# lucasjinreal/yolov7_d2

Hardware: NVIDIA H100
Metric: images/sec (640x640) YOLOX-s fwd+bwd (higher is better)
Workload: dtype bf16

## Files before the change

yolov7_d2_b200/csrc/conv_api.cu:

```cuda
#include "conv_gemm.cuh"
#include "host_common.cuh"
#include "wgrad_gemm.cuh"

#include <algorithm>
#include <cstring>

namespace yb {

template <int BN, int BK>
static int launch_conv_inst(const CUtensorMap& tmA, const CUtensorMap& tmB, const ConvGemmParams& p, dim3 grid, cudaStream_t st) {
  using Cfg = ConvGemmCfg<BN, BK>;
  const bool ext = p.epi_mode >= EPI_BF16_AFFINE;
  const int phases = p.num_phases == 4 ? 4 : 1;
  const int m_tiles = grid.x * phases, n_tiles = grid.y;
  const int occ = conv_min_ctas(BN, BK);
  const bool xpose = p.epi_mode == EPI_F32_BIAS && p.out_sc == 1;
  const int fixed = ConvEpiCfg<BN>::kStageBytes + (xpose ? kXposeBytes : 0);
  const int budget = (occ == 1 ? 212 : 104) * 1024 - 1024 - fixed;
  int slots_kb = budget / Cfg::kStageBytes;
  const int num_kb = phases == 4 ? p.cin_blocks : p.num_taps * p.cin_blocks;
  int kbs = 1;
  if (BK <= 32)
    for (int t = 1; t <= num_kb; ++t)
      if (num_kb % t == 0 && t * BK <= 144 && 2 * t <= slots_kb) kbs = t;
  int pst = slots_kb / kbs;
  if (pst > kMaxStagesP) pst = kMaxStagesP;
  if (pst < 2) pst = 2;
  const int smem = pst * kbs * Cfg::kStageBytes + 1024 + fixed;
  static PerDevice<int> smem_limit(0);
  YB_CHECK_CUDA(raise_smem_limit(smem_limit, smem, conv_gemm_persistent_kernel<BN, BK, false>, conv_gemm_persistent_kernel<BN, BK, true>));
  int groups = (occ * sm_count()) / n_tiles;
  if (groups < 1) groups = 1;
  if (groups > m_tiles) groups = m_tiles;
  if (phases == 4 && groups > 1 && groups % 2 == 0) --groups;
  ConvGemmParams pp = p;
  pp.xpose = xpose ? 1 : 0;
  if (ext)
    launch_k(conv_gemm_persistent_kernel<BN, BK, true>, groups * n_tiles, kConvThreadsP, smem, st, tmA, tmB, pp, pst, kbs, n_tiles, m_tiles);
  else
    launch_k(conv_gemm_persistent_kernel<BN, BK, false>, groups * n_tiles, kConvThreadsP, smem, st, tmA, tmB, pp, pst, kbs, n_tiles, m_tiles);
  YB_CHECK_CUDA(cudaGetLastError());
  return 0;
}

static int launch_conv(int bn, int bk, const CUtensorMap& tmA, const CUtensorMap& tmB, const ConvGemmParams& p, dim3 grid, cudaStream_t st) {
#define YB_CASE(BN, BK) \
  if (bn == BN && bk == BK) return launch_conv_inst<BN, BK>(tmA, tmB, p, grid, st);
  YB_CASE(16, 16) YB_CASE(16, 32) YB_CASE(16, 64)
  YB_CASE(32, 16) YB_CASE(32, 32) YB_CASE(32, 64)
  YB_CASE(64, 16) YB_CASE(64, 32) YB_CASE(64, 64)
  YB_CASE(128, 16) YB_CASE(128, 32) YB_CASE(128, 64)
#undef YB_CASE
  return fail(YB200_ERR_UNSUPPORTED, "no conv_gemm instantiation for BLOCK_N=%d BLOCK_K=%d", bn, bk);
}

static int pick_block_k(int c) { return c % 64 == 0 ? 64 : (c % 32 == 0 ? 32 : (c % 16 == 0 ? 16 : 0)); }
static int pick_block_n(int c) { return c > 64 ? 128 : (c > 32 ? 64 : (c > 16 ? 32 : 16)); }

static int check_arg(const yb200_act* a, const char* who, const char* arg) {
  char name[96];
  snprintf(name, sizeof(name), "%s %s", who, arg);
  return check_act(a, name);
}

static int fill_fwd_taps(ConvTap* taps, const yb200_act& x, int ksize, int stride, int k_per_tap) {
  int nt = 0;
  if (ksize == 1) {
    taps[nt++] = ConvTap{x.c_off, 0, 0, 0, 0};
  } else if (ksize == 2) {
    for (int kh = 0; kh < 2; ++kh)
      for (int kw = 0; kw < 2; ++kw) taps[nt++] = ConvTap{kw * x.c_pitch + x.c_off, 0, kh, 0, (kh * 2 + kw) * k_per_tap};
  } else {
    for (int kh = 0; kh < 3; ++kh)
      for (int kw = 0; kw < 3; ++kw) {
        ConvTap t{};
        if (stride == 1) {
          t.c0 = x.c_off; t.dw = kw - 1; t.p = 0; t.dh = kh - 1;
        } else {
          t.p = (kh == 1) ? 0 : 1; t.dh = (kh == 0) ? -1 : 0;
          const int pw = (kw == 1) ? 0 : 1;
          t.dw = (kw == 0) ? -1 : 0;
          t.c0 = pw * x.c_pitch + x.c_off;
        }
        t.kb = (kh * 3 + kw) * k_per_tap;
        taps[nt++] = t;
      }
  }
  return nt;
}

static ConvGemmParams out_view(const yb200_act& o) {
  ConvGemmParams p;
  memset(&p, 0, sizeof(p));
  p.out = static_cast<__nv_bfloat16*>(o.ptr) + o.c_off;
  p.out_sw = o.c_pitch;
  p.out_sh = 1LL * o.c_pitch * o.w;
  p.out_sn = 1LL * o.c_pitch * o.w * o.h;
  p.out_sc = 1;
  p.out_mh = 1; p.out_mw = 1;
  return p;
}
static ConvGemmParams out_rows_f32(float* out, int w, int a_total, int a_off, int c_total, int c_off) {
  ConvGemmParams p;
  memset(&p, 0, sizeof(p));
  p.out = out + 1LL * a_off * c_total + c_off;
  p.out_sn = 1LL * a_total * c_total;
  p.out_sh = 1LL * w * c_total;
  p.out_sw = c_total;
  p.out_sc = 1;
  p.out_mh = 1; p.out_mw = 1;
  return p;
}
static ConvGemmParams out_nchw_f32(float* out, int cout, int h, int w) {
  ConvGemmParams p;
  memset(&p, 0, sizeof(p));
  const long long hw = 1LL * h * w;
  p.out = out;
  p.out_sn = 1LL * cout * hw;
  p.out_sh = w;
  p.out_sw = 1;
  p.out_sc = static_cast<int>(hw);
  p.out_mh = 1; p.out_mw = 1;
  return p;
}
static ConvGemmParams out_nhwc_f32(float* out, int pitch, int h, int w) {
  ConvGemmParams p;
  memset(&p, 0, sizeof(p));
  p.out = out;
  p.out_sw = pitch;
  p.out_sh = 1LL * pitch * w;
  p.out_sn = 1LL * pitch * w * h;
  p.out_sc = 1;
  p.out_mh = 1; p.out_mw = 1;
  return p;
}

static void set_addend(ConvGemmParams& p, const yb200_act* a) {
  p.addend = static_cast<const __nv_bfloat16*>(a->ptr) + a->c_off;
  p.add_sw = a->c_pitch;
  p.add_sh = 1LL * a->c_pitch * a->w;
  p.add_sn = 1LL * a->c_pitch * a->w * a->h;
}

static void set_tiles(ConvGemmParams& p, int n, int h, int w) {
  choose_tile(n, h, w, 128, &p.log_tw, &p.log_th);
  const int tw = 1 << p.log_tw, th = 1 << p.log_th, tn = 128 >> (p.log_tw + p.log_th);
  p.tiles_w = ceil_div(w, tw); p.tiles_h = ceil_div(h, th); p.tiles_n = ceil_div(n, tn);
  p.n_valid = n; p.h_valid = h; p.w_valid = w;
}

}

using namespace yb;

__global__ void pack_conv_weight_kernel(const float* __restrict__ w, const float* __restrict__ cout_scale, int cout, int cin, int taps, int cout_pad,
                                        int cin_pad, __nv_bfloat16* __restrict__ wf, __nv_bfloat16* __restrict__ wd) {
  pdl_sync();
  const long long total = 1LL * cout_pad * taps * cin_pad;
  for (long long i = blockIdx.x * (long long)blockDim.x + threadIdx.x; i < total; i += (long long)gridDim.x * blockDim.x) {
    const int ci = static_cast<int>(i % cin_pad);
    const int t = static_cast<int>((i / cin_pad) % taps);
    const int co = static_cast<int>(i / (1LL * cin_pad * taps));
    float v = (co < cout && ci < cin) ? w[(1LL * co * cin + ci) * taps + t] : 0.f;
    if (cout_scale != nullptr && co < cout) v *= cout_scale[co];
    const __nv_bfloat16 b = __float2bfloat16_rn(v);
    if (wf) wf[i] = b;
    if (wd) wd[(1LL * ci * taps + t) * cout_pad + co] = b;
  }
}

static int pack_weight_impl(const float* w_oihw, const float* cout_scale, int cout, int cin, int ksize, int cout_pad, int cin_pad, void* w_fwd,
                            void* w_dgrad, void* stream) {
  YB_REQUIRE(w_oihw && (w_fwd || w_dgrad), YB200_ERR_INVALID, "pack_conv_weight: null pointer");
  YB_REQUIRE(cout > 0 && cin > 0 && (ksize >= 1 && ksize <= 3) && cout_pad >= cout && cin_pad >= cin, YB200_ERR_INVALID,
             "pack_conv_weight: bad sizes cout=%d cin=%d k=%d pads=%d,%d", cout, cin, ksize, cout_pad, cin_pad);
  const long long total = 1LL * cout_pad * ksize * ksize * cin_pad;
  const int blocks = static_cast<int>(std::min<long long>((total + 255) / 256, 4096));
  launch_k(pack_conv_weight_kernel, blocks, 256, 0, as_stream(stream), w_oihw, cout_scale, cout, cin, ksize * ksize, cout_pad, cin_pad,
                                                                 static_cast<__nv_bfloat16*>(w_fwd),
                                                                 static_cast<__nv_bfloat16*>(w_dgrad));
  YB_CHECK_CUDA(cudaGetLastError());
  return 0;
}

constexpr int kPackMaxLayers = 256;
__global__ void __launch_bounds__(256)
pack_conv_weights_batched_kernel(const yb200_pack_desc* __restrict__ table, const long long* __restrict__ prefix, int n) {
  pdl_sync();
  __shared__ int s_rows[kPackMaxLayers + 1];
  if (threadIdx.x == 0) {
    int acc = 0;
    for (int l = 0; l < n; ++l) {
      s_rows[l] = acc;
      const yb200_pack_desc d = table[l];
      const int taps = d.ksize * d.ksize;
      acc += (d.w_fwd ? d.cout_pad * taps : 0) + (d.w_dgrad ? d.cin_pad * taps : 0);
    }
    s_rows[n] = acc;
  }
  __syncthreads();
  const int total_rows = s_rows[n];
  const int lane = threadIdx.x & 31;
  const int warps = (gridDim.x * blockDim.x) >> 5;
  for (int r = (blockIdx.x * blockDim.x + threadIdx.x) >> 5; r < total_rows; r += warps) {
    int lo = 0, hi = n - 1;
    while (lo < hi) {
      const int mid = (lo + hi + 1) >> 1;
      if (s_rows[mid] <= r) lo = mid; else hi = mid - 1;
    }
    const yb200_pack_desc d = table[lo];
    const int taps = d.ksize * d.ksize;
    int q = r - s_rows[lo];
    const int fwd_rows = d.w_fwd ? d.cout_pad * taps : 0;
    if (q < fwd_rows) {
      const int co = q / taps, t = q - co * taps;
      __nv_bfloat16* dst = static_cast<__nv_bfloat16*>(d.w_fwd) + static_cast<size_t>(q) * d.cin_pad;
      const float* src = d.w_oihw + static_cast<size_t>(co) * d.cin * taps + t;
      for (int ci = lane; ci < d.cin_pad; ci += 32)
        dst[ci] = __float2bfloat16_rn((co < d.cout && ci < d.cin) ? src[static_cast<size_t>(ci) * taps] : 0.f);
    } else {
      q -= fwd_rows;
      const int ci = q / taps, t = q - ci * taps;
      __nv_bfloat16* dst = static_cast<__nv_bfloat16*>(d.w_dgrad) + static_cast<size_t>(q) * d.cout_pad;
      const float* src = d.w_oihw + static_cast<size_t>(ci) * taps + t;
      for (int co = lane; co < d.cout_pad; co += 32)
        dst[co] = __float2bfloat16_rn((co < d.cout && ci < d.cin) ? src[static_cast<size_t>(co) * d.cin * taps] : 0.f);
    }
  }
}

extern "C" int yb200_pack_conv_weights_batched(const yb200_pack_desc* table_dev, const int64_t* prefix_dev, int n, int64_t total, void* stream) {
  YB_REQUIRE(table_dev && prefix_dev && n > 0 && n <= kPackMaxLayers && total > 0, YB200_ERR_INVALID, "pack_conv_weights_batched: bad arguments (n=%d)", n);
  const int blocks = static_cast<int>(std::min<long long>((2 * total + 255) / 256, 16LL * sm_count()));
  launch_k(pack_conv_weights_batched_kernel, blocks, 256, 0, as_stream(stream), table_dev, reinterpret_cast<const long long*>(prefix_dev), n);
  YB_CHECK_CUDA(cudaGetLastError());
  return 0;
}

extern "C" int yb200_pack_conv_weight(const float* w_oihw, int cout, int cin, int ksize, int cout_pad, int cin_pad, void* w_fwd,
                                      void* w_dgrad, void* stream) {
  return pack_weight_impl(w_oihw, nullptr, cout, cin, ksize, cout_pad, cin_pad, w_fwd, w_dgrad, stream);
}

__global__ void scale_bias_kernel(const float* __restrict__ scale, const float* __restrict__ bias, int n, float* __restrict__ out) {
  pdl_sync();
  const int i = blockIdx.x * blockDim.x + threadIdx.x;
  if (i < n) out[i] = scale[i] * bias[i];
}

extern "C" int yb200_pack_conv_weight_scaled(const float* w_oihw, const float* cout_scale, const float* bias, int cout, int cin, int ksize,
                                             int cout_pad, int cin_pad, void* w_fwd, void* w_dgrad, float* scaled_bias, void* stream) {
  YB_REQUIRE(cout_scale != nullptr, YB200_ERR_INVALID, "pack_conv_weight_scaled: null scale");
  YB_REQUIRE((bias == nullptr) == (scaled_bias == nullptr), YB200_ERR_INVALID, "pack_conv_weight_scaled: pass both bias and scaled_bias or neither");
  if (bias) launch_k(scale_bias_kernel, ceil_div(cout, 256), 256, 0, as_stream(stream), cout_scale, bias, cout, scaled_bias);
  return pack_weight_impl(w_oihw, cout_scale, cout, cin, ksize, cout_pad, cin_pad, w_fwd, w_dgrad, stream);
}

static void expand_split_taps(ConvGemmParams& p, int c, int lo_delta, int planes) {
  const int nt = p.num_taps;
  const int plane_kb = nt * c;
  int terms[6][2], nterm = 0;
  for (int sum = 0; sum < planes; ++sum)
    for (int i = 0; i <= sum; ++i) { terms[nterm][0] = i; terms[nterm][1] = sum - i; ++nterm; }
  for (int t = nt - 1; t >= 0; --t) {
    const ConvTap b = p.taps[t];
    for (int q = 0; q < nterm; ++q) {
      ConvTap e = b;
      e.c0 = b.c0 + terms[q][0] * lo_delta;
      e.kb = b.kb + terms[q][1] * plane_kb;
      p.taps[nterm * t + q] = e;
    }
  }
  p.num_taps = nterm * nt;
}

static int conv_fwd_common(const char* who, const yb200_act* x, const void* w_fwd, long long w_rows, int cout, int ksize, int stride,
                           ConvGemmParams& p, cudaStream_t st, int lo_delta = 0, int planes = 1, int group = 0) {
  YB_REQUIRE(w_fwd != nullptr, YB200_ERR_INVALID, "%s: null weights", who);
  YB_REQUIRE((ksize == 1 && stride == 1) || (ksize == 2 && stride == 2) || (ksize == 3 && (stride == 1 || stride == 2)), YB200_ERR_UNSUPPORTED,
             "%s: ksize=%d stride=%d not implemented", who, ksize, stride);
  const int bk = pick_block_k(x->c);
  YB_REQUIRE(bk != 0, YB200_ERR_UNSUPPORTED, "%s: input channels %d must be a multiple of 16", who, x->c);
  const int bn = pick_block_n(cout);
  const int oh = x->h / stride, ow = x->w / stride;
  set_tiles(p, x->n, oh, ow);
  p.num_taps = fill_fwd_taps(p.taps, *x, ksize, stride, x->c);
  long long kcols = 1LL * p.num_taps * x->c;
  if (lo_delta > 0) {
    YB_REQUIRE(planes == 2 || planes == 3, YB200_ERR_INVALID, "%s: %d planes", who, planes);
    YB_REQUIRE(lo_delta % 8 == 0 && x->c_off + (planes - 1) * lo_delta + x->c <= x->c_pitch, YB200_ERR_INVALID,
               "%s: plane %d [%d, %d) outside the channel pitch %d", who, planes - 1, x->c_off + (planes - 1) * lo_delta,
               x->c_off + (planes - 1) * lo_delta + x->c, x->c_pitch);
    expand_split_taps(p, x->c, lo_delta, planes);
    kcols *= planes;
  }
  p.cin_blocks = x->c / bk;
  p.cout = cout;
  if (group > 1 && ksize == 3 && stride == 1 && lo_delta == 0 && p.cin_blocks == 1 && x->c_off == 0 && x->c == x->c_pitch && (x->c / group) % 16 == 0) {
    const int cpp = x->c / group;
    for (int t = 0; t < p.num_taps; ++t) {
      ConvTap& tp = p.taps[t];
      if (tp.dw == -1) { tp.c0 += (group - 1) * cpp; tp.kb += (group - 1) * cpp; }
    }
  }
  const int tw = 1 << p.log_tw, th = 1 << p.log_th, tn = 128 >> (p.log_tw + p.log_th);
  CUtensorMap tmA, tmB;
  int rc = make_act_map(&tmA, *x, stride == 2, bk, tw, th, tn);
  if (rc) return rc;
  rc = make_mat_map(&tmB, w_fwd, w_rows, kcols, bn, bk);
  if (rc) return rc;
  dim3 grid(p.tiles_w * p.tiles_h * p.tiles_n, ceil_div(cout, bn));
  return launch_conv(bn, bk, tmA, tmB, p, grid, st);
}

static int check_fwd(const char* who, const yb200_act* x, const yb200_act* out, const char* out_name, const yb200_act* residual, int stride) {
  int rc;
  if ((rc = check_arg(x, who, "x"))) return rc;
  if ((rc = check_arg(out, who, out_name))) return rc;
  if (residual && (rc = check_arg(residual, who, "residual"))) return rc;
  YB_REQUIRE(stride == 1 || stride == 2, YB200_ERR_UNSUPPORTED, "%s: stride %d", who, stride);
  YB_REQUIRE(out->n == x->n && out->h * stride == x->h && out->w * stride == x->w, YB200_ERR_INVALID,
             "%s: output %dx%dx%d does not match input %dx%dx%d / stride %d", who, out->n, out->h, out->w, x->n, x->h, x->w, stride);
  YB_REQUIRE(!residual || same_shape(residual, out), YB200_ERR_INVALID, "%s: residual shape mismatch", who);
  return 0;
}

static int conv2d_fwd_impl(const char* who, const yb200_act* x, const void* w_fwd, const yb200_act* z, int ksize, int stride, double* stat_sum,
                           double* stat_sqsum, int stat_fold, void* stream) {
  int rc;
  if ((rc = check_fwd(who, x, z, "z", nullptr, stride))) return rc;
  YB_REQUIRE((stat_sum == nullptr) == (stat_sqsum == nullptr), YB200_ERR_INVALID, "%s: pass both or neither stat buffer", who);
  ConvGemmParams p = out_view(*z);
  p.epi_mode = stat_sum ? EPI_F16_STATS : EPI_F16;
  p.stat_sum = stat_sum;
  p.stat_sq = stat_sqsum;
  p.stat_fold = stat_fold;
  return conv_fwd_common(who, x, w_fwd, z->c, z->c, ksize, stride, p, as_stream(stream), 0, 1, stat_fold > 0 ? z->c / stat_fold : 0);
}

extern "C" int yb200_conv2d_fwd(const yb200_act* x, const void* w_fwd, const yb200_act* z, int ksize, int stride,
                                double* stat_sum, double* stat_sqsum, void* stream) {
  return conv2d_fwd_impl("conv2d_fwd", x, w_fwd, z, ksize, stride, stat_sum, stat_sqsum, 0, stream);
}
// ... 396 lines not shown
```

yolov7_d2_b200/csrc/conv_gemm.cuh:

```cuda
#pragma once
#include <cuda_fp16.h>

#include "sm90.cuh"

namespace yb {

constexpr int kMaxTaps = 54;

enum EpiMode : int {
  EPI_BF16 = 0,
  EPI_F16 = 1,
  EPI_F16_STATS = 2,
  EPI_F32_BIAS = 3,
  EPI_BF16_BN_SILU = 4,
  EPI_BF16_AFFINE = 5,
  EPI_BF16_BIAS_GELU = 6,
  EPI_BF16_GELU_BWD = 7,
  EPI_BF16_BIAS_RELU = 8,
  EPI_BF16_RELU_BWD = 9,
};

__device__ __forceinline__ bool epi_has_stats(int mode, const double* stat_sum) {
  return mode == EPI_F16_STATS || ((mode == EPI_BF16_GELU_BWD || mode == EPI_BF16_RELU_BWD) && stat_sum != nullptr);
}
__device__ __forceinline__ float gelu_phi(float u, float& e) {
  const float z = fabsf(u) * 0.70710678118654752f;
  const float t = __fdividef(1.f, fmaf(0.3275911f, z, 1.f));
  const float poly = t * fmaf(t, fmaf(t, fmaf(t, fmaf(t, 1.061405429f, -1.453152027f), 1.421413741f), -0.284496736f), 0.254829592f);
  e = __expf(-z * z);
  const float q = 0.5f * poly * e;
  return u >= 0.f ? 1.f - q : q;
}
__device__ __forceinline__ float gelu_erf(float u) {
  float e;
  return u * gelu_phi(u, e);
}
__device__ __forceinline__ float gelu_erf_grad(float u) {
  float e;
  const float phi = gelu_phi(u, e);
  return fmaf(u * 0.3989422804014327f, e, phi);
}

struct ConvTap {
  int c0;
  int dw;
  int p;
  int dh;
  int kb;
  int ks;
};

struct ConvGemmParams {
  int tiles_w, tiles_h, tiles_n;
  int log_tw, log_th;
  int num_taps, cin_blocks;
  int n_valid, h_valid, w_valid;
  int cout;
  int epi_mode;
  long long out_sn, out_sh, out_sw;
  int out_sc, out_mh, out_mw;
  void* out;
  const __nv_bfloat16* addend;
  long long add_sn, add_sh, add_sw;
  const float* bias;
  const float* scale;
  const float* shift;
  double* stat_sum;
  double* stat_sq;
  int stat_fold;
  int num_phases;
  int phase_tap[5];
  int b_img_rows;
  int xpose;
  const __nv_bfloat16* aux_in;
  __nv_bfloat16* aux_out;
  ConvTap taps[kMaxTaps];
};

__device__ __forceinline__ void conv_decode_work(const ConvGemmParams& p, int wi, int& m, int& tap0, int& ntaps, int& oph, int& opw) {
  if (p.num_phases == 4) {
    m = wi >> 2;
    const int ph = wi & 3;
    tap0 = p.phase_tap[ph];
    ntaps = p.phase_tap[ph + 1] - tap0;
    oph = ph >> 1;
    opw = ph & 1;
  } else {
    m = wi; tap0 = 0; ntaps = p.num_taps; oph = opw = 0;
  }
}

template <int BLOCK_N, int BLOCK_K>
struct ConvGemmCfg {
  static constexpr int kSwizzle = BLOCK_K * 2;
  static constexpr int kABytes = 128 * BLOCK_K * 2;
  static constexpr int kBBytes = BLOCK_N * BLOCK_K * 2;
  static constexpr int kStageBytes = kABytes + kBBytes;
  static_assert(BLOCK_K == 16 || BLOCK_K == 32 || BLOCK_K == 64, "BLOCK_K");
  static_assert(BLOCK_N == 16 || BLOCK_N == 32 || BLOCK_N == 64 || BLOCK_N == 128, "BLOCK_N");
  static_assert(kABytes % (8 * kSwizzle) == 0 && kStageBytes % (8 * kSwizzle) == 0, "tiles must start on a swizzle-pattern boundary");
};

__device__ __forceinline__ uint32_t pack_f16x2(float lo, float hi) {
  __half2 v = __floats2half2_rn(lo, hi);
  return *reinterpret_cast<uint32_t*>(&v);
}
__device__ __forceinline__ void store_f16x8(__half* dst, const float* v) {
  uint4 u;
  u.x = pack_f16x2(v[0], v[1]);
  u.y = pack_f16x2(v[2], v[3]);
  u.z = pack_f16x2(v[4], v[5]);
  u.w = pack_f16x2(v[6], v[7]);
  *reinterpret_cast<uint4*>(dst) = u;
}
__device__ __forceinline__ void store_bf16x8(__nv_bfloat16* dst, const float* v) {
  uint4 u;
  u.x = pack_bf16x2(v[0], v[1]);
  u.y = pack_bf16x2(v[2], v[3]);
  u.z = pack_bf16x2(v[4], v[5]);
  u.w = pack_bf16x2(v[6], v[7]);
  *reinterpret_cast<uint4*>(dst) = u;
}

template <int BLOCK_N>
__device__ __forceinline__ void stage_col_params(const ConvGemmParams& p, int col0, float (*s_col)[BLOCK_N]) {
  const float* sh = p.shift ? p.shift : p.bias;
  for (int i = threadIdx.x; i < BLOCK_N; i += blockDim.x) {
    const bool ok = col0 + i < p.cout;
    s_col[0][i] = (ok && p.scale) ? p.scale[col0 + i] : 1.f;
    s_col[1][i] = (ok && sh) ? sh[col0 + i] : 0.f;
  }
}

constexpr int kXposeWarpFloats = 32 * 33 + 64;
constexpr int kXposeBytes = 8 * kXposeWarpFloats * 4;

template <int CH, bool EXT = true>
__device__ __forceinline__ void conv_epilogue_chunk(const ConvGemmParams& p, float (&v)[CH], bool valid, long long pix_off, long long add_off,
                                                    int cbase, int lane, float* part_sum, float* part_sq, bool accumulate,
                                                    const float* col_scale, const float* col_shift, float* xp = nullptr) {
  if (p.epi_mode == EPI_F32_BIAS) {
    if (xp != nullptr) {
      long long* s_off = reinterpret_cast<long long*>(xp + 32 * 33);
#pragma unroll
      for (int i = 0; i < CH; ++i) xp[lane * 33 + i] = v[i] + col_shift[i];
      s_off[lane] = valid ? pix_off : -1;
      __syncwarp();
      float* o = reinterpret_cast<float*>(p.out) + cbase + lane;
      const bool colok = lane < CH && cbase + lane < p.cout;
#pragma unroll 8
      for (int r = 0; r < 32; ++r) {
        const long long off = s_off[r];
        if (off >= 0 && colok) o[off] = xp[r * 33 + lane];
      }
      __syncwarp();
      return;
    }
    if (valid) {
      float* o = reinterpret_cast<float*>(p.out) + pix_off;
#pragma unroll
      for (int i = 0; i < CH; ++i)
        if (cbase + i < p.cout) o[(long long)(cbase + i) * p.out_sc] = v[i] + col_shift[i];
    }
    return;
  }
  if (p.epi_mode == EPI_BF16_BN_SILU) {
#pragma unroll
    for (int i = 0; i < CH; i += 4) {
      const float4 sc = *reinterpret_cast<const float4*>(col_scale + i), sh = *reinterpret_cast<const float4*>(col_shift + i);
      const float u0 = fmaf(v[i], sc.x, sh.x), u1 = fmaf(v[i + 1], sc.y, sh.y), u2 = fmaf(v[i + 2], sc.z, sh.z), u3 = fmaf(v[i + 3], sc.w, sh.w);
      v[i] = bf16_round(__fdividef(u0, 1.f + __expf(-u0)));
      v[i + 1] = bf16_round(__fdividef(u1, 1.f + __expf(-u1)));
      v[i + 2] = bf16_round(__fdividef(u2, 1.f + __expf(-u2)));
      v[i + 3] = bf16_round(__fdividef(u3, 1.f + __expf(-u3)));
    }
  }
  if constexpr (EXT) {
    if (p.epi_mode == EPI_BF16_AFFINE) {
      if (p.scale != nullptr) {
  #pragma unroll
        for (int i = 0; i < CH; i += 4) {
          const float4 sc = *reinterpret_cast<const float4*>(col_scale + i);
          v[i] *= sc.x; v[i + 1] *= sc.y; v[i + 2] *= sc.z; v[i + 3] *= sc.w;
        }
      }
      if (p.shift != nullptr) {
  #pragma unroll
        for (int i = 0; i < CH; i += 4) {
          const float4 sh = *reinterpret_cast<const float4*>(col_shift + i);
          v[i] += sh.x; v[i + 1] += sh.y; v[i + 2] += sh.z; v[i + 3] += sh.w;
        }
      }
    }
    if (p.epi_mode == EPI_BF16_BIAS_RELU) {
  #pragma unroll
      for (int i = 0; i < CH; i += 4) {
        const float4 sh = *reinterpret_cast<const float4*>(col_shift + i);
        v[i] = fmaxf(v[i] + sh.x, 0.f); v[i + 1] = fmaxf(v[i + 1] + sh.y, 0.f);
        v[i + 2] = fmaxf(v[i + 2] + sh.z, 0.f); v[i + 3] = fmaxf(v[i + 3] + sh.w, 0.f);
      }
    }
    if (p.epi_mode == EPI_BF16_RELU_BWD && valid) {
      const __nv_bfloat16* a = p.aux_in + pix_off + cbase;
  #pragma unroll
      for (int i = 0; i < CH; i += 8) {
        if (cbase + i < p.cout) {
          const uint4 u = *reinterpret_cast<const uint4*>(a + i);
          v[i + 0] = (u.x & 0xFFFFu) - 1u < 0x7FFFu ? v[i + 0] : 0.f; v[i + 1] = (u.x >> 16) - 1u < 0x7FFFu ? v[i + 1] : 0.f;
          v[i + 2] = (u.y & 0xFFFFu) - 1u < 0x7FFFu ? v[i + 2] : 0.f; v[i + 3] = (u.y >> 16) - 1u < 0x7FFFu ? v[i + 3] : 0.f;
          v[i + 4] = (u.z & 0xFFFFu) - 1u < 0x7FFFu ? v[i + 4] : 0.f; v[i + 5] = (u.z >> 16) - 1u < 0x7FFFu ? v[i + 5] : 0.f;
          v[i + 6] = (u.w & 0xFFFFu) - 1u < 0x7FFFu ? v[i + 6] : 0.f; v[i + 7] = (u.w >> 16) - 1u < 0x7FFFu ? v[i + 7] : 0.f;
        }
      }
    }
    if (p.epi_mode == EPI_BF16_BIAS_GELU) {
  #pragma unroll
      for (int i = 0; i < CH; i += 4) {
        const float4 sh = *reinterpret_cast<const float4*>(col_shift + i);
        v[i] = bf16_round(v[i] + sh.x); v[i + 1] = bf16_round(v[i + 1] + sh.y);
        v[i + 2] = bf16_round(v[i + 2] + sh.z); v[i + 3] = bf16_round(v[i + 3] + sh.w);
      }
      if (p.aux_out != nullptr && valid) {
        __nv_bfloat16* o = p.aux_out + pix_off + cbase;
  #pragma unroll
        for (int i = 0; i < CH; i += 8)
          if (cbase + i < p.cout) store_bf16x8(o + i, v + i);
      }
  #pragma unroll
      for (int i = 0; i < CH; ++i) v[i] = gelu_erf(v[i]);
    }
    if (p.epi_mode == EPI_BF16_GELU_BWD && valid) {
      const __nv_bfloat16* a = p.aux_in + pix_off + cbase;
  #pragma unroll
      for (int i = 0; i < CH; i += 8) {
        if (cbase + i < p.cout) {
          const uint4 u = *reinterpret_cast<const uint4*>(a + i);
          v[i + 0] *= gelu_erf_grad(bf16_lo(u.x)); v[i + 1] *= gelu_erf_grad(bf16_hi(u.x));
          v[i + 2] *= gelu_erf_grad(bf16_lo(u.y)); v[i + 3] *= gelu_erf_grad(bf16_hi(u.y));
          v[i + 4] *= gelu_erf_grad(bf16_lo(u.z)); v[i + 5] *= gelu_erf_grad(bf16_hi(u.z));
          v[i + 6] *= gelu_erf_grad(bf16_lo(u.w)); v[i + 7] *= gelu_erf_grad(bf16_hi(u.w));
        }
      }
    }
  }
  if (p.addend != nullptr && valid) {
    const __nv_bfloat16* a = p.addend + add_off + cbase;
#pragma unroll
    for (int i = 0; i < CH; i += 8) {
      if (cbase + i < p.cout) {
        const uint4 u = *reinterpret_cast<const uint4*>(a + i);
        v[i + 0] += bf16_lo(u.x); v[i + 1] += bf16_hi(u.x);
        v[i + 2] += bf16_lo(u.y); v[i + 3] += bf16_hi(u.y);
        v[i + 4] += bf16_lo(u.z); v[i + 5] += bf16_hi(u.z);
        v[i + 6] += bf16_lo(u.w); v[i + 7] += bf16_hi(u.w);
      }
    }
  }
  const bool f16 = p.epi_mode == EPI_F16 || p.epi_mode == EPI_F16_STATS;
  const bool need_vals = p.epi_mode == EPI_F16_STATS || (EXT && p.stat_sum != nullptr);
  if (f16) {
    uint32_t pk[CH / 2];
#pragma unroll
    for (int i = 0; i < CH; i += 2) pk[i >> 1] = pack_f16x2(v[i], v[i + 1]);
    if (valid) {
      __half* o = reinterpret_cast<__half*>(p.out) + pix_off + cbase;
#pragma unroll
      for (int i = 0; i < CH; i += 8)
        if (cbase + i < p.cout) *reinterpret_cast<uint4*>(o + i) = make_uint4(pk[i >> 1], pk[(i >> 1) + 1], pk[(i >> 1) + 2], pk[(i >> 1) + 3]);
    }
    if (need_vals) {
#pragma unroll
      for (int i = 0; i < CH; i += 2) {
        __half2 h;
        *reinterpret_cast<uint32_t*>(&h) = pk[i >> 1];
        const float2 f = __half22float2(h);
        v[i] = valid ? f.x : 0.f;
        v[i + 1] = valid ? f.y : 0.f;
      }
    }
  } else {
    uint32_t pk[CH / 2];
#pragma unroll
    for (int i = 0; i < CH; i += 2) pk[i >> 1] = pack_bf16x2(v[i], v[i + 1]);
    if (valid) {
      __nv_bfloat16* o = reinterpret_cast<__nv_bfloat16*>(p.out) + pix_off + cbase;
#pragma unroll
      for (int i = 0; i < CH; i += 8)
        if (cbase + i < p.cout) *reinterpret_cast<uint4*>(o + i) = make_uint4(pk[i >> 1], pk[(i >> 1) + 1], pk[(i >> 1) + 2], pk[(i >> 1) + 3]);
    }
    if (need_vals) {
#pragma unroll
      for (int i = 0; i < CH; i += 2) {
        v[i] = valid ? bf16_lo(pk[i >> 1]) : 0.f;
        v[i + 1] = valid ? bf16_hi(pk[i >> 1]) : 0.f;
      }
    }
  }
  if (p.epi_mode == EPI_F16_STATS) {
    float sq[CH];
#pragma unroll
    for (int i = 0; i < CH; ++i) sq[i] = v[i] * v[i];
    float cs, cq;
    if constexpr (CH == 32) { cs = warp_colsum32(v, lane); cq = warp_colsum32(sq, lane); }
    else { cs = warp_colsum16(v, lane); cq = warp_colsum16(sq, lane); }
    if (lane < CH) {
      part_sum[lane] = accumulate ? part_sum[lane] + cs : cs;
      part_sq[lane] = accumulate ? part_sq[lane] + cq : cq;
    }
  } else if (EXT && (p.epi_mode == EPI_BF16_GELU_BWD || p.epi_mode == EPI_BF16_RELU_BWD) && p.stat_sum != nullptr) {
    float cs;
    if constexpr (CH == 32) cs = warp_colsum32(v, lane);
    else cs = warp_colsum16(v, lane);
    if (lane < CH) part_sum[lane] = accumulate ? part_sum[lane] + cs : cs;
  }
}

constexpr int kMaxStagesP = 8;
constexpr int kConvThreadsP = 288;

template <int BLOCK_N>
struct ConvEpiCfg {
  static constexpr int kCols = BLOCK_N <= 64 ? (BLOCK_N < 32 ? BLOCK_N : 32) : 64;
  static_assert(BLOCK_N % kCols == 0, "staging rounds must cover the column tile");
  static constexpr int kPitch = kCols + 4;
  static constexpr int kHalves = BLOCK_N >= 32 ? 2 : 1;
  static constexpr int kChunk = kCols / kHalves;
  static constexpr int kStageBytes = 2 * 64 * kPitch * 4;
};

__host__ __device__ constexpr int conv_min_ctas(int block_n, int block_k) { return (block_n >= 128 || block_k == 16) ? 1 : 2; }

template <int BLOCK_N, int BLOCK_K, bool EXT>
__global__ void __launch_bounds__(kConvThreadsP, conv_min_ctas(BLOCK_N, BLOCK_K))
conv_gemm_persistent_kernel(const __grid_constant__ CUtensorMap tmA, const __grid_constant__ CUtensorMap tmB,
                            const __grid_constant__ ConvGemmParams p, int num_stages, int kb_per_slot, int n_tiles, int m_tiles) {
  using Cfg = ConvGemmCfg<BLOCK_N, BLOCK_K>;
  using Epi = ConvEpiCfg<BLOCK_N>;
  constexpr int CH = Epi::kChunk;
  extern __shared__ uint8_t smem_dyn[];
  __shared__ __align__(8) uint64_t s_bar[2 * kMaxStagesP];
  __shared__ float s_part[4][2][BLOCK_N];
  __shared__ __align__(16) float s_col[2][BLOCK_N];

  const int warp = warp_id_uniform();
  const int lane = threadIdx.x & 31;
  const uint32_t smem_base = (smem_u32(smem_dyn) + 1023u) & ~1023u;
  uint8_t* const smem_al = smem_dyn + (smem_base - smem_u32(smem_dyn));
  const int ring_bytes = num_stages * kb_per_slot * Cfg::kStageBytes;
  const uint32_t bar_full = smem_u32(&s_bar[0]);
  const uint32_t bar_empty = smem_u32(&s_bar[kMaxStagesP]);

  const int n_tile = blockIdx.x % n_tiles;
  const int group = blockIdx.x / n_tiles;
  const int groups = gridDim.x / n_tiles;
  const int col0 = n_tile * BLOCK_N;
  const int log_tw = p.log_tw, log_th = p.log_th;

  if (threadIdx.x == 0) {
    for (int s = 0; s < num_stages; ++s) {
      mbar_init(bar_full + 8 * s, 1);
      mbar_init(bar_empty + 8 * s, 2);
    }
    mbar_fence_init();
  }
  for (int i = threadIdx.x; i < 4 * 2 * BLOCK_N; i += blockDim.x) (&s_part[0][0][0])[i] = 0.f;
  pdl_sync();
  stage_col_params<BLOCK_N>(p, col0, s_col);
  __syncthreads();

  if (warp == 8) {
    if (elect_one()) {
      tma_prefetch_desc(&tmA);
      tma_prefetch_desc(&tmB);
      int stage = 0;
      uint32_t phase = 0;
      for (int wi = group; wi < m_tiles; wi += groups) {
        int m, tap, ntaps, oph, opw;
        conv_decode_work(p, wi, m, tap, ntaps, oph, opw);
        const int num_kb = ntaps * p.cin_blocks;
        int t = m;
        const int tw = t % p.tiles_w;
        t /= p.tiles_w;
        const int th = t % p.tiles_h;
        const int tn = t / p.tiles_h;
        const int w0 = tw << log_tw, h0 = th << log_th, n0 = tn << (7 - log_tw - log_th);
        int cb = 0;
        for (int kb = 0; kb < num_kb; kb += kb_per_slot) {
          mbar_wait(bar_empty + 8 * stage, phase ^ 1u);
          const uint32_t full = bar_full + 8 * stage;
          mbar_expect_tx(full, Cfg::kStageBytes * kb_per_slot);
          for (int j = 0; j < kb_per_slot; ++j) {
            const uint32_t sa = smem_base + (stage * kb_per_slot + j) * Cfg::kStageBytes;
            const ConvTap& tp = p.taps[tap];
            tma_load_5d(sa, &tmA, full, tp.c0 + cb * BLOCK_K, w0 + tp.dw, tp.p, h0 + tp.dh, n0);
            tma_load_2d(sa + Cfg::kABytes, &tmB, full, tp.kb + cb * BLOCK_K, col0 + n0 * p.b_img_rows);
            if (++cb == p.cin_blocks) { cb = 0; ++tap; }
          }
          if (++stage == num_stages) { stage = 0; phase ^= 1u; }
        }
      }
    }
  } else if (warp < 8) {
    const int g = warp >> 2;
    const int wl = warp & 3;
    const int q = 2 * g + (wl & 1);
    const int half = wl >> 1;
    const int mrow = q * 32 + lane;
    const int xl = mrow & ((1 << log_tw) - 1);
    const int yl = (mrow >> log_tw) & ((1 << log_th) - 1);
    const int nl = mrow >> (log_tw + log_th);
    float* const stg = reinterpret_cast<float*>(smem_al + ring_bytes) + g * 64 * Epi::kPitch;
    float* xp = nullptr;
    if (p.xpose) xp = reinterpret_cast<float*>(smem_al + ring_bytes + Epi::kStageBytes) + warp * kXposeWarpFloats;
    constexpr uint32_t lcode = gmma_layout_code(Cfg::kSwizzle);
    constexpr uint32_t sbo = 8 * Cfg::kSwizzle;
    float acc[BLOCK_N / 2];
#pragma unroll
    for (int i = 0; i < BLOCK_N / 2; ++i) acc[i] = 0.f;
    wgmma_fence_operand(acc);
    int stage = 0;
    uint32_t phase = 0;
    for (int wi = group; wi < m_tiles; wi += groups) {
      int m, tap, ntaps, oph, opw;
      conv_decode_work(p, wi, m, tap, ntaps, oph, opw);
      const int num_kb = ntaps * p.cin_blocks;
      int j = 0, prev = -1;
      for (int kb = 0; kb < num_kb; ++kb) {
        if (j == 0) mbar_wait(bar_full + 8 * stage, phase);
        const uint32_t sa = smem_base + (stage * kb_per_slot + j) * Cfg::kStageBytes + g * 64 * Cfg::kSwizzle;
        const uint32_t sb = smem_base + (stage * kb_per_slot + j) * Cfg::kStageBytes + Cfg::kABytes;
        wgmma_fence_operand(acc);
        wgmma_fence();
#pragma unroll
        for (int k = 0; k < BLOCK_K / 16; ++k)
          Wgmma<BLOCK_N>::template mma<0, 0>(acc, gmma_desc(sa + k * 32, 16, sbo, lcode), gmma_desc(sb + k * 32, 16, sbo, lcode), (kb | k) != 0 ? 1u : 0u);
        wgmma_commit();
        wgmma_wait<1>();
        wgmma_fence_operand(acc);
        mbar_arrive_if(bar_empty + 8 * prev, j == 0 && prev >= 0 && (threadIdx.x & 127) == 0);
        if (++j == kb_per_slot) {
          j = 0;
          prev = stage;
          if (++stage == num_stages) { stage = 0; phase ^= 1u; }
        }
      }
      wgmma_wait<0>();
      wgmma_fence_operand(acc);
      mbar_arrive_if(bar_empty + 8 * prev, (threadIdx.x & 127) == 0);

      int t = m;
      const int tw = t % p.tiles_w;
      t /= p.tiles_w;
      const int th = t % p.tiles_h;
      const int tn = t / p.tiles_h;
      const int x = (tw << log_tw) + xl, y = (th << log_th) + yl, n = (tn << (7 - log_tw - log_th)) + nl;
      const bool valid = (x < p.w_valid) && (y < p.h_valid) && (n < p.n_valid);
      const long long pix_off = (long long)n * p.out_sn + (long long)(y * p.out_mh + oph) * p.out_sh +
                                (long long)(x * p.out_mw + opw) * p.out_sw;
      const long long add_off = (long long)n * p.add_sn + (long long)(y * p.out_mh + oph) * p.add_sh +
                                (long long)(x * p.out_mw + opw) * p.add_sw;
      float* const r0 = stg + (16 * wl + (lane >> 2)) * Epi::kPitch + 2 * (lane & 3);
      float* const r1 = r0 + 8 * Epi::kPitch;
      const float* const row_src = stg + ((wl & 1) * 32 + lane) * Epi::kPitch + half * CH;
#pragma unroll 1
      for (int r = 0; r < BLOCK_N / Epi::kCols; ++r) {
        named_bar_sync(1 + g, 128);
#pragma unroll
        for (int i = 0; i < BLOCK_N / 8; ++i) {
          if (i / (Epi::kCols / 8) == r) {
            const int c = (i % (Epi::kCols / 8)) * 8;
            *reinterpret_cast<float2*>(r0 + c) = make_float2(acc[4 * i], acc[4 * i + 1]);
            *reinterpret_cast<float2*>(r1 + c) = make_float2(acc[4 * i + 2], acc[4 * i + 3]);
          }
        }
        named_bar_sync(1 + g, 128);
        const int c = r * Epi::kCols + half * CH;
        if (half < Epi::kHalves && col0 + c < p.cout) {
          float v[CH];
#pragma unroll
          for (int i = 0; i < CH; i += 4) {
            const float4 f = *reinterpret_cast<const float4*>(row_src + i);
            v[i] = f.x; v[i + 1] = f.y; v[i + 2] = f.z; v[i + 3] = f.w;
          }
          conv_epilogue_chunk<CH, EXT>(p, v, valid, pix_off, add_off, col0 + c, lane, &s_part[q][0][c], &s_part[q][1][c], true, &s_col[0][c],
                                       &s_col[1][c], xp);
        }
      }
    }
  }

  __syncthreads();
  if (EXT ? epi_has_stats(p.epi_mode, p.stat_sum) : p.epi_mode == EPI_F16_STATS) {
    for (int e = threadIdx.x; e < BLOCK_N && col0 + e < p.cout; e += blockDim.x) {
      const float s1 = (s_part[0][0][e] + s_part[1][0][e]) + (s_part[2][0][e] + s_part[3][0][e]);
      const float s2 = (s_part[0][1][e] + s_part[1][1][e]) + (s_part[2][1][e] + s_part[3][1][e]);
      const int ch = p.stat_fold > 0 ? (col0 + e) % p.stat_fold : col0 + e;
      atomicAdd(p.stat_sum + ch, static_cast<double>(s1));
      if (p.stat_sq != nullptr) atomicAdd(p.stat_sq + ch, static_cast<double>(s2));
    }
  }
}

}
```

yolov7_d2_b200/csrc/host_common.cu:

```cuda
#include "host_common.cuh"

#include <mutex>

namespace yb {

static thread_local char g_err[1024] = "";

char* err_buf() { return g_err; }

int fail(int code, const char* fmt, ...) {
  va_list ap;
  va_start(ap, fmt);
  vsnprintf(g_err, sizeof(g_err), fmt, ap);
  va_end(ap);
  return code;
}

int current_device() {
  int dev = 0;
  if (cudaGetDevice(&dev) != cudaSuccess) return 0;
  return dev;
}

int sm_count() {
  static int n[64] = {0};
  const int dev = current_device() & 63;
  if (n[dev] == 0) {
    if (cudaDeviceGetAttribute(&n[dev], cudaDevAttrMultiProcessorCount, dev) != cudaSuccess || n[dev] <= 0) n[dev] = 132;
  }
  return n[dev];
}

int check_act(const yb200_act* a, const char* name, int mult) {
  YB_REQUIRE(a != nullptr && a->ptr != nullptr, YB200_ERR_INVALID, "%s: null view", name);
  YB_REQUIRE(a->n > 0 && a->h > 0 && a->w > 0 && a->c > 0, YB200_ERR_INVALID, "%s: empty extent (%dx%dx%dx%d)", name, a->n, a->h, a->w, a->c);
  YB_REQUIRE(a->c % mult == 0 && a->c_pitch % mult == 0 && a->c_off % mult == 0 && a->c_off + a->c <= a->c_pitch, YB200_ERR_INVALID,
             "%s: channels (c=%d pitch=%d off=%d) must be multiples of %d with off+c<=pitch", name, a->c, a->c_pitch, a->c_off, mult);
  return 0;
}

typedef CUresult (*EncodeTiledFn)(CUtensorMap*, CUtensorMapDataType, cuuint32_t, void*, const cuuint64_t*,
                                  const cuuint64_t*, const cuuint32_t*, const cuuint32_t*, CUtensorMapInterleave,
                                  CUtensorMapSwizzle, CUtensorMapL2promotion, CUtensorMapFloatOOBfill);

static EncodeTiledFn encode_fn() {
  static EncodeTiledFn fn = nullptr;
  static std::once_flag once;
  std::call_once(once, [] {
    void* p = nullptr;
    cudaDriverEntryPointQueryResult q;
    if (cudaGetDriverEntryPoint("cuTensorMapEncodeTiled", &p, cudaEnableDefault, &q) == cudaSuccess &&
        q == cudaDriverEntryPointSuccess)
      fn = reinterpret_cast<EncodeTiledFn>(p);
  });
  return fn;
}

static CUtensorMapSwizzle swizzle_for(int inner_bytes) {
  return inner_bytes == 128 ? CU_TENSOR_MAP_SWIZZLE_128B
         : inner_bytes == 64 ? CU_TENSOR_MAP_SWIZZLE_64B
         : inner_bytes == 32 ? CU_TENSOR_MAP_SWIZZLE_32B
                             : CU_TENSOR_MAP_SWIZZLE_NONE;
}

int make_act_map(CUtensorMap* m, const yb200_act& a, bool s2d, int box_c, int tw, int th, int tn) {
  EncodeTiledFn fn = encode_fn();
  YB_REQUIRE(fn != nullptr, YB200_ERR_CUDA, "cuTensorMapEncodeTiled entry point not available");
  YB_REQUIRE(box_c == 16 || box_c == 32 || box_c == 64, YB200_ERR_INVALID, "activation box width %d", box_c);
  YB_REQUIRE((reinterpret_cast<uintptr_t>(a.ptr) & 15) == 0 && a.c_pitch % 8 == 0, YB200_ERR_INVALID,
             "activation buffer must be 16B aligned with a channel pitch multiple of 8");
  const cuuint64_t pitch = static_cast<cuuint64_t>(a.c_pitch) * 2;
  cuuint64_t gdim[5], gstr[4];
  if (!s2d) {
    gdim[0] = a.c_pitch; gdim[1] = a.w; gdim[2] = 1; gdim[3] = a.h; gdim[4] = a.n;
    gstr[0] = pitch; gstr[1] = pitch * a.w; gstr[2] = pitch * a.w; gstr[3] = pitch * a.w * a.h;
  } else {
    YB_REQUIRE(a.h % 2 == 0 && a.w % 2 == 0, YB200_ERR_UNSUPPORTED, "stride-2 view needs even h,w (got %dx%d)", a.h, a.w);
    gdim[0] = 2 * a.c_pitch; gdim[1] = a.w / 2; gdim[2] = 2; gdim[3] = a.h / 2; gdim[4] = a.n;
    gstr[0] = 2 * pitch; gstr[1] = pitch * a.w; gstr[2] = 2 * pitch * a.w; gstr[3] = pitch * a.w * a.h;
  }
  cuuint32_t box[5] = {static_cast<cuuint32_t>(box_c), static_cast<cuuint32_t>(tw), 1u, static_cast<cuuint32_t>(th),
                       static_cast<cuuint32_t>(tn)};
  cuuint32_t estr[5] = {1, 1, 1, 1, 1};
  CUresult r = fn(m, CU_TENSOR_MAP_DATA_TYPE_BFLOAT16, 5, a.ptr, gdim, gstr, box, estr, CU_TENSOR_MAP_INTERLEAVE_NONE,
                  swizzle_for(box_c * 2), CU_TENSOR_MAP_L2_PROMOTION_L2_128B, CU_TENSOR_MAP_FLOAT_OOB_FILL_NONE);
  YB_REQUIRE(r == CUDA_SUCCESS, YB200_ERR_CUDA,
             "cuTensorMapEncodeTiled(act n=%d h=%d w=%d pitch=%d box=%d,%d,%d,%d) failed: %d", a.n, a.h, a.w, a.c_pitch,
             box_c, tw, th, tn, static_cast<int>(r));
  return 0;
}

int make_mat_map(CUtensorMap* m, const void* ptr, long long rows, long long cols, int box_rows, int box_cols) {
  EncodeTiledFn fn = encode_fn();
  YB_REQUIRE(fn != nullptr, YB200_ERR_CUDA, "cuTensorMapEncodeTiled entry point not available");
  YB_REQUIRE((reinterpret_cast<uintptr_t>(ptr) & 15) == 0 && cols % 8 == 0, YB200_ERR_INVALID,
             "matrix must be 16B aligned with a row length multiple of 8");
  cuuint64_t gdim[2] = {static_cast<cuuint64_t>(cols), static_cast<cuuint64_t>(rows)};
  cuuint64_t gstr[1] = {static_cast<cuuint64_t>(cols) * 2};
  cuuint32_t box[2] = {static_cast<cuuint32_t>(box_cols), static_cast<cuuint32_t>(box_rows)};
  cuuint32_t estr[2] = {1, 1};
  CUresult r = fn(m, CU_TENSOR_MAP_DATA_TYPE_BFLOAT16, 2, const_cast<void*>(ptr), gdim, gstr, box, estr,
                  CU_TENSOR_MAP_INTERLEAVE_NONE, swizzle_for(box_cols * 2), CU_TENSOR_MAP_L2_PROMOTION_L2_128B,
                  CU_TENSOR_MAP_FLOAT_OOB_FILL_NONE);
  YB_REQUIRE(r == CUDA_SUCCESS, YB200_ERR_CUDA, "cuTensorMapEncodeTiled(mat %lldx%lld box %dx%d) failed: %d", rows, cols,
             box_rows, box_cols, static_cast<int>(r));
  return 0;
}

void choose_tile(int n, int h, int w, int npix, int* log_tw, int* log_th) {
  const int lp = ilog2(npix);
  long long best = -1;
  int bw = 0, bh = 0;
  for (int lw = lp; lw >= 0; --lw) {
    for (int lh = lp - lw; lh >= 0; --lh) {
      const int tw = 1 << lw, th = 1 << lh, tn = npix >> (lw + lh);
      const long long cost = 1LL * ceil_div(w, tw) * tw * ceil_div(h, th) * th * ceil_div(n, tn) * tn;
      if (best < 0 || cost < best) {
        best = cost; bw = lw; bh = lh;
      }
    }
  }
  *log_tw = bw;
  *log_th = bh;
}

}

extern "C" int yb200_version(void) { return YB200_VERSION; }
extern "C" const char* yb200_last_error(void) { return yb::err_buf(); }
```

yolov7_d2_b200/csrc/host_common.cuh:

```cuda
#pragma once
#include <cuda.h>
#include <cuda_runtime.h>
#include <stdarg.h>
#include <stdio.h>
#include <string.h>

#include <utility>

#include "../../include/yb200.h"

namespace yb {

char* err_buf();
int fail(int code, const char* fmt, ...);
int sm_count();
int current_device();
template <typename T>
struct PerDevice {
  T v[64];
  T init;
  bool used[64];
  explicit PerDevice(T init_value) : init(init_value) { memset(used, 0, sizeof(used)); }
  T& cur() {
    const int d = current_device() & 63;
    if (!used[d]) { v[d] = init; used[d] = true; }
    return v[d];
  }
};

template <typename... K>
inline cudaError_t raise_smem_limit(PerDevice<int>& limit, int bytes, K*... kernels) {
  int& cur = limit.cur();
  if (bytes <= cur) return cudaSuccess;
  cudaError_t e = cudaSuccess;
  ((e = e == cudaSuccess ? cudaFuncSetAttribute(kernels, cudaFuncAttributeMaxDynamicSharedMemorySize, bytes) : e), ...);
  if (e == cudaSuccess) cur = bytes;
  return e;
}

#define YB_CHECK_CUDA(expr)                                                                      \
  do {                                                                                           \
    cudaError_t _e = (expr);                                                                     \
    if (_e != cudaSuccess) return yb::fail(YB200_ERR_CUDA, "%s: %s", #expr, cudaGetErrorString(_e)); \
  } while (0)
#define YB_REQUIRE(cond, code, ...) \
  do {                              \
    if (!(cond)) return yb::fail(code, __VA_ARGS__); \
  } while (0)

inline cudaStream_t as_stream(void* s) { return reinterpret_cast<cudaStream_t>(s); }

int check_act(const yb200_act* a, const char* name, int mult = 8);
inline bool same_shape(const yb200_act* a, const yb200_act* b) { return a->n == b->n && a->h == b->h && a->w == b->w && a->c == b->c; }
inline bool same_geometry(const yb200_act* a, const yb200_act* b) { return same_shape(a, b) && a->c_pitch == b->c_pitch; }

int make_act_map(CUtensorMap* m, const yb200_act& a, bool space_to_depth, int box_c, int tw, int th, int tn);
int make_mat_map(CUtensorMap* m, const void* ptr, long long rows, long long cols, int box_rows, int box_cols);

void choose_tile(int n, int h, int w, int npix, int* log_tw, int* log_th);

template <typename... K, typename... A>
inline cudaError_t launch_k_opt(bool pdl, void (*kernel)(K...), dim3 grid, dim3 block, size_t smem, cudaStream_t st, A&&... args) {
  cudaLaunchConfig_t cfg = {};
  cfg.gridDim = grid;
  cfg.blockDim = block;
  cfg.dynamicSmemBytes = smem;
  cfg.stream = st;
  cudaLaunchAttribute at[1];
  at[0].id = cudaLaunchAttributeProgrammaticStreamSerialization;
  at[0].val.programmaticStreamSerializationAllowed = 1;
  cfg.attrs = at;
  cfg.numAttrs = pdl ? 1 : 0;
  return cudaLaunchKernelEx(&cfg, kernel, std::forward<A>(args)...);
}
template <typename... K, typename... A>
inline cudaError_t launch_k(void (*kernel)(K...), dim3 grid, dim3 block, size_t smem, cudaStream_t st, A&&... args) {
  return launch_k_opt(true, kernel, grid, block, smem, st, std::forward<A>(args)...);
}

inline int ceil_div(int a, int b) { return (a + b - 1) / b; }
inline int ilog2(int v) { int l = 0; while ((1 << l) < v) ++l; return l; }

}
```

Measured before the change: 2053.

## Use atomic work-stealing counters for persistent conv GEMM tile scheduling

The producer warp now claims M tiles dynamically from a per-stream, per-column-tile global atomic counter instead of a static strided assignment. It passes each claimed tile index to the MMA warps through a shared array guarded by the pipeline barriers, and uses a sentinel to signal termination. The last finisher resets the counter so it can be reused. The goal is to balance load across persistent CTAs when tiles have uneven cost, such as multi-phase or variable-tap work. In exchange it adds atomic latency per tile, consumes an extra pipeline stage slot for termination, and depends on the counter reset being correct across back-to-back launches on the same stream. Kernels that accumulate stats keep the static schedule.

```diff
diff --git a/yolov7_d2_b200/csrc/conv_api.cu b/yolov7_d2_b200/csrc/conv_api.cu
--- a/yolov7_d2_b200/csrc/conv_api.cu
+++ b/yolov7_d2_b200/csrc/conv_api.cu
@@ -33,12 +33,17 @@
   if (groups < 1) groups = 1;
   if (groups > m_tiles) groups = m_tiles;
   if (phases == 4 && groups > 1 && groups % 2 == 0) --groups;
+  int* work_ctr = nullptr;
+  if (!epi_has_stats(p.epi_mode, p.stat_sum)) {
+    const int rc = work_counters(st, n_tiles, &work_ctr);
+    if (rc) return rc;
+  }
   ConvGemmParams pp = p;
   pp.xpose = xpose ? 1 : 0;
   if (ext)
-    launch_k(conv_gemm_persistent_kernel<BN, BK, true>, groups * n_tiles, kConvThreadsP, smem, st, tmA, tmB, pp, pst, kbs, n_tiles, m_tiles);
+    launch_k(conv_gemm_persistent_kernel<BN, BK, true>, groups * n_tiles, kConvThreadsP, smem, st, tmA, tmB, pp, pst, kbs, n_tiles, m_tiles, work_ctr);
   else
-    launch_k(conv_gemm_persistent_kernel<BN, BK, false>, groups * n_tiles, kConvThreadsP, smem, st, tmA, tmB, pp, pst, kbs, n_tiles, m_tiles);
+    launch_k(conv_gemm_persistent_kernel<BN, BK, false>, groups * n_tiles, kConvThreadsP, smem, st, tmA, tmB, pp, pst, kbs, n_tiles, m_tiles, work_ctr);
   YB_CHECK_CUDA(cudaGetLastError());
   return 0;
 }
diff --git a/yolov7_d2_b200/csrc/conv_gemm.cuh b/yolov7_d2_b200/csrc/conv_gemm.cuh
--- a/yolov7_d2_b200/csrc/conv_gemm.cuh
+++ b/yolov7_d2_b200/csrc/conv_gemm.cuh
@@ -20,7 +20,7 @@
   EPI_BF16_RELU_BWD = 9,
 };
 
-__device__ __forceinline__ bool epi_has_stats(int mode, const double* stat_sum) {
+__host__ __device__ __forceinline__ bool epi_has_stats(int mode, const double* stat_sum) {
   return mode == EPI_F16_STATS || ((mode == EPI_BF16_GELU_BWD || mode == EPI_BF16_RELU_BWD) && stat_sum != nullptr);
 }
 __device__ __forceinline__ float gelu_phi(float u, float& e) {
@@ -333,12 +333,13 @@
 template <int BLOCK_N, int BLOCK_K, bool EXT>
 __global__ void __launch_bounds__(kConvThreadsP, conv_min_ctas(BLOCK_N, BLOCK_K))
 conv_gemm_persistent_kernel(const __grid_constant__ CUtensorMap tmA, const __grid_constant__ CUtensorMap tmB,
-                            const __grid_constant__ ConvGemmParams p, int num_stages, int kb_per_slot, int n_tiles, int m_tiles) {
+                            const __grid_constant__ ConvGemmParams p, int num_stages, int kb_per_slot, int n_tiles, int m_tiles, int* work_ctr) {
   using Cfg = ConvGemmCfg<BLOCK_N, BLOCK_K>;
   using Epi = ConvEpiCfg<BLOCK_N>;
   constexpr int CH = Epi::kChunk;
   extern __shared__ uint8_t smem_dyn[];
   __shared__ __align__(8) uint64_t s_bar[2 * kMaxStagesP];
+  __shared__ int s_item[kMaxStagesP];
   __shared__ float s_part[4][2][BLOCK_N];
   __shared__ __align__(16) float s_col[2][BLOCK_N];
 
@@ -372,9 +373,18 @@
     if (elect_one()) {
       tma_prefetch_desc(&tmA);
       tma_prefetch_desc(&tmB);
+      int* const ctr = work_ctr != nullptr ? work_ctr + n_tile : nullptr;
       int stage = 0;
       uint32_t phase = 0;
-      for (int wi = group; wi < m_tiles; wi += groups) {
+      int wi = ctr != nullptr ? atomicAdd(ctr, 1) : group;
+      for (;;) {
+        mbar_wait(bar_empty + 8 * stage, phase ^ 1u);
+        s_item[stage] = wi;
+        if (wi >= m_tiles) {
+          if (ctr != nullptr && wi == m_tiles + groups - 1) atomicExch(ctr, 0);
+          mbar_arrive(bar_full + 8 * stage);
+          break;
+        }
         int m, tap, ntaps, oph, opw;
         conv_decode_work(p, wi, m, tap, ntaps, oph, opw);
         const int num_kb = ntaps * p.cin_blocks;
@@ -386,7 +396,7 @@
         const int w0 = tw << log_tw, h0 = th << log_th, n0 = tn << (7 - log_tw - log_th);
         int cb = 0;
         for (int kb = 0; kb < num_kb; kb += kb_per_slot) {
-          mbar_wait(bar_empty + 8 * stage, phase ^ 1u);
+          if (kb > 0) mbar_wait(bar_empty + 8 * stage, phase ^ 1u);
           const uint32_t full = bar_full + 8 * stage;
           mbar_expect_tx(full, Cfg::kStageBytes * kb_per_slot);
           for (int j = 0; j < kb_per_slot; ++j) {
@@ -398,6 +408,7 @@
           }
           if (++stage == num_stages) { stage = 0; phase ^= 1u; }
         }
+        wi = ctr != nullptr ? atomicAdd(ctr, 1) : wi + groups;
       }
     }
   } else if (warp < 8) {
@@ -420,7 +431,10 @@
     wgmma_fence_operand(acc);
     int stage = 0;
     uint32_t phase = 0;
-    for (int wi = group; wi < m_tiles; wi += groups) {
+    for (;;) {
+      mbar_wait(bar_full + 8 * stage, phase);
+      const int wi = s_item[stage];
+      if (wi >= m_tiles) break;
       int m, tap, ntaps, oph, opw;
       conv_decode_work(p, wi, m, tap, ntaps, oph, opw);
       const int num_kb = ntaps * p.cin_blocks;
diff --git a/yolov7_d2_b200/csrc/host_common.cu b/yolov7_d2_b200/csrc/host_common.cu
--- a/yolov7_d2_b200/csrc/host_common.cu
+++ b/yolov7_d2_b200/csrc/host_common.cu
@@ -1,5 +1,6 @@
 #include "host_common.cuh"
 
+#include <map>
 #include <mutex>
 
 namespace yb {
@@ -29,6 +30,29 @@
     if (cudaDeviceGetAttribute(&n[dev], cudaDevAttrMultiProcessorCount, dev) != cudaSuccess || n[dev] <= 0) n[dev] = 132;
   }
   return n[dev];
+}
+
+constexpr int kWorkCtrStreams = 128;
+constexpr int kWorkCtrSlots = 512;
+__device__ int g_work_ctr[kWorkCtrStreams * kWorkCtrSlots];
+
+int work_counters(cudaStream_t st, int n, int** out) {
+  YB_REQUIRE(n > 0 && n <= kWorkCtrSlots, YB200_ERR_UNSUPPORTED, "work_counters: %d column tiles (at most %d)", n, kWorkCtrSlots);
+  static std::mutex mu;
+  static std::map<std::pair<int, cudaStream_t>, int> slot_of;
+  static int used[64];
+  static int* base[64];
+  const int dev = current_device() & 63;
+  std::lock_guard<std::mutex> lock(mu);
+  if (base[dev] == nullptr) YB_CHECK_CUDA(cudaGetSymbolAddress(reinterpret_cast<void**>(&base[dev]), g_work_ctr));
+  auto it = slot_of.find({dev, st});
+  if (it == slot_of.end()) {
+    YB_REQUIRE(used[dev] < kWorkCtrStreams, YB200_ERR_UNSUPPORTED, "work_counters: convolutions launched on more than %d streams of device %d",
+               kWorkCtrStreams, dev);
+    it = slot_of.emplace(std::make_pair(dev, st), used[dev]++).first;
+  }
+  *out = base[dev] + it->second * kWorkCtrSlots;
+  return 0;
 }
 
 int check_act(const yb200_act* a, const char* name, int mult) {
diff --git a/yolov7_d2_b200/csrc/host_common.cuh b/yolov7_d2_b200/csrc/host_common.cuh
--- a/yolov7_d2_b200/csrc/host_common.cuh
+++ b/yolov7_d2_b200/csrc/host_common.cuh
@@ -54,6 +54,8 @@
 inline bool same_shape(const yb200_act* a, const yb200_act* b) { return a->n == b->n && a->h == b->h && a->w == b->w && a->c == b->c; }
 inline bool same_geometry(const yb200_act* a, const yb200_act* b) { return same_shape(a, b) && a->c_pitch == b->c_pitch; }
 
+int work_counters(cudaStream_t st, int n, int** out);
+
 int make_act_map(CUtensorMap* m, const yb200_act& a, bool space_to_depth, int box_c, int tw, int th, int tn);
 int make_mat_map(CUtensorMap* m, const void* ptr, long long rows, long long cols, int box_rows, int box_cols);
 
```

Measured after the change: 2058, median of 6. Within noise of the previous version (+0.2%).
